# uncbiag/OAI_analysis_2

Hardware: AMD Instinct MI355X
Metric: knee MRI volumes/sec (segment+register), 384x384x160 fp32 (higher is better)
Workload: dtype fp16x3 (every fp32 value held as 2 fp16 terms = 22 mantissa bits, 3 MFMA passes per product, fp32 accumulate; fp32 in and out of every entry point; full-size parity vs the reference in `parity`)

## Files before the change

oai_analysis_2_amd/csrc/unet.hip:

```cpp
#include <cmath>
#include <cstdint>
#include <cstdlib>
#include <cstring>
#include <algorithm>
#include <vector>

#include "unet_host.h"
#include "unet_wino.h"

#ifdef OAI_DIAG
static unsigned long long* g_diag_stamps = nullptr;
static unsigned long long* diag_stamps() {
    if (!g_diag_stamps && oai::diag_env("OAI_STAMPS", 0)) {
        if (hipMalloc((void**)&g_diag_stamps, 32 * sizeof(unsigned long long)) != hipSuccess) return nullptr;
        (void)hipMemset(g_diag_stamps, 0, 32 * sizeof(unsigned long long));
    }
    return g_diag_stamps;
}
extern "C" int oai_diag_stamps(unsigned long long out[32], int reset) {
    if (!g_diag_stamps) return 1;
    if (hipMemcpy(out, g_diag_stamps, 32 * sizeof(unsigned long long), hipMemcpyDeviceToHost) != hipSuccess) return 2;
    if (reset) (void)hipMemset(g_diag_stamps, 0, 32 * sizeof(unsigned long long));
    return 0;
}
// ... 221 lines not shown
    return best;
}


int fill_conv_args(const oai_unet* h, const Layer& L, const float* s0, const float* s1, float* out, const int dims[3], const ConvOpt& o, ConvArgs& a) {
    if (o.head) a = *o.head;
    if (o.store_boxes && h->sres && h->opt_dead_stores) { a.store_boxes = o.store_boxes; a.store_grow = 1; }
    if (o.first) {
        a.first_w = h->L[EC0].plain; a.first_scale = h->L[EC0].scale_f16; a.first_shift = h->L[EC0].shift_f16; a.first_src = *o.first;
        a.first_census = census_of(h, EC0);
    }
    if (const Scatter* sc = o.sc) {
        a.sc_boxes = sc->boxes; a.sc_ntiles = sc->ntiles; a.sc_tile0 = sc->tile0;
        for (int i = 0; i < 3; ++i) { a.sc_g[i] = sc->g[i]; a.sc_e[i] = sc->e[i]; a.sc_t[i] = sc->t[i]; }
    }
    a.boxes = o.boxes;
    a.pool_out = o.pool_out;
    a.range_flag = h->range_flag;
#ifdef OAI_DIAG
    a.stamps = layer_stamps(h, L);
#endif
    a.src0 = s0; a.src1 = s1; a.C0 = L.c0; a.C1 = s1 ? L.c1 : 0;
    const bool f16 = h->precision == OAI_PREC_FP16X3;
    a.out = out; a.Cout = L.cout; a.scale = f16 ? L.scale_f16 : L.scale; a.shift = f16 ? L.shift_f16 : L.shift;
    a.census = h->sres ? census_of(h, layer_id(h, L)) : nullptr;
    a.wpanel = h->precision == OAI_PREC_F32 ? L.panel : L.panel_bf[h->precision == OAI_PREC_BF16X3 ? 0 : h->precision == OAI_PREC_BF16X6 ? 1 : 2];
    a.wpanel16 = h->precision == OAI_PREC_FP16X3 && layer_bit(h, h->opt_m16_layers, L) ? L.panel_m16 : nullptr;
    a.D = dims[0]; a.H = dims[1]; a.W = dims[2];
    a.ncb = (L.cout + 63) / 64;
    a.relu = 1;
// ... 9 lines not shown
    if (h->precision == OAI_PREC_F32 && h->variant == 0 && h->opt_wino_f32 && L.panel_wino_f32 && a.Cout % 4 == 0 && !a.head_w && !a.first_w && !a.sc_boxes &&
        (!a.pool_out || (wino_pool_box(box, dims) && dims[0] % 2 == 0)) && layer_bit(h, h->opt_wino_layers, L))
        return launch_conv3_wino_f32(h, L, a, box, ntiles, st);
    if (h->sres && h->opt_wino && L.panel_wino && h->sres_mrep == 4 && !a.first_w && !a.head_w && !a.sc_boxes &&
        (!a.pool_out || (a.Cout % 128 == 0 && a.relu && wino_pool_box(box, dims))) && a.Cout % 64 == 0 && (h->opt_wino & (a.Cout % 128 == 0 ? 1 : 2)) && (a.Cout % 128 == 0 || (a.C0 + 15) / 16 + (a.C1 + 15) / 16 >= 8) && layer_bit(h, h->opt_wino_layers, L) && (size_t)dims[0] * dims[1] * dims[2] < (1u << 24))
        return launch_conv3_wino(h, L, a, box, ntiles, st, o.oc);
    return launch_conv3_direct(h, a, box, ntiles, st);
}

static bool pool_fusable(const oai_unet* h, const int dims[3], const Box& box) {
    if (h->variant != 0) return false;
    for (int i = 0; i < 3; ++i) if (box.lo[i] != 0 || box.hi[i] != dims[i]) return false;
    return dims[0] % 4 == 0 && dims[1] % 8 == 0 && dims[2] % 16 == 0;
}


static int run_batch(oai_unet* h, const TileSource& src, int n, const Box need[18], int out_mode,
                     float* blocks_out, float* const buf[B_COUNT], hipStream_t st,
                     const int* table = nullptr, int table_tiles = 0, int t0 = 0, const SharedEnc* se = nullptr, const OwnPlan* own = nullptr) {
    auto tb = [&](int layer) -> const int* { return table ? table + ((size_t)layer * table_tiles + t0) * 6 : nullptr; };
    if (!table || !h->opt_own_cover) own = nullptr;
    OwnCover ocs[kOwnLayers];
    auto oc = [&](int layer) -> const OwnCover* {
        if (!own) return nullptr;
        const int slot = own_cover_slot(layer);
        ocs[slot].list = own->list[slot]; ocs[slot].list_len = own->list_len[slot];
        for (int s = 0; s < 3; ++s) {
            ocs[slot].rows[s] = tb(18 + 3 * slot + s);
            for (int i = 0; i < 3; ++i) ocs[slot].nb[s][i] = own->nb[slot][s][i];
            const int ncb = h->L[layer].cout / (64 * wino_groups(h, h->L[layer].cout, kWinoTY[s]));
            ocs[slot].xcd_group[s] = own->nb[slot][s][0] && ncb > 0 && !ocs[slot].list_len ? balanced_xcd_group(h->xcd_group, own->tile_nb.data() + (slot * 3 + s) * 3, n, own->nb[slot][s], ncb) : 0;
        }
        return &ocs[slot];
    };
    auto upv = [&](int layer) { return own ? own->up_nvox[layer] : 0; };
    const Layer* L = h->L;
    int d[4][3];
    for (int l = 0; l < 4; ++l) { d[l][0] = src.td >> l; d[l][1] = src.th >> l; d[l][2] = src.tw >> l; }

    int rc;
#define RUN(x) do { rc = (x); if (rc) return rc; } while (0)
    if (se) {
        {
            TileSource vs{};
            vs.vol = se->vol; vs.D = se->D; vs.H = se->H; vs.W = se->W; vs.td = se->PD; vs.th = se->PH; vs.tw = se->PW;
            vs.ez = se->PD; vs.ey = se->PH; vs.ex = se->PW; vs.oz = se->overlap[0]; vs.oy = se->overlap[1]; vs.ox = se->overlap[2]; vs.gy = 1; vs.gx = 1;
            const int per_row = se->grid[1] * se->grid[2], P[3] = {se->PD, se->PH, se->PW};
            Scatter sc;
            sc.boxes = tb(DC2); sc.ntiles = n; sc.tile0 = src.tile_begin;
            for (int i = 0; i < 3; ++i) { sc.g[i] = se->grid[i]; sc.e[i] = se->eff[i]; }
            sc.t[0] = src.td; sc.t[1] = src.th; sc.t[2] = src.tw;
            const int t_first = src.tile_begin, t_last = src.tile_begin + n - 1;
            const int zspan = (src.td + se->eff[0] - 1) / se->eff[0];
            const int s_first = t_first / per_row, s_last = t_last / per_row + zspan - 1;
            Box prev{}; bool have_prev = false;
            for (int s = s_first; s <= s_last; ++s) {
// ... 10 lines not shown
                if (jhi < 0) continue;
                Box bx;
                bx.lo[0] = se->eff[0] * s; bx.hi[0] = std::min(P[0], se->eff[0] * (s + 1));
                if (s == s_last) bx.hi[0] = std::min(P[0], se->eff[0] * (t_last / per_row) + src.td);
                bx.lo[1] = se->eff[1] * jlo; bx.hi[1] = std::min(P[1], se->eff[1] * jhi + src.th);
                bx.lo[2] = se->eff[2] * klo; bx.hi[2] = std::min(P[2], se->eff[2] * khi + src.tw);
                if (have_prev && prev.lo[1] == bx.lo[1] && prev.hi[1] == bx.hi[1] && prev.lo[2] == bx.lo[2] && prev.hi[2] == bx.hi[2] && prev.hi[0] == bx.lo[0]) {
                    prev.hi[0] = bx.hi[0];
                    continue;
                }
                if (have_prev) RUN(launch_conv3(h, L[EC1], nullptr, nullptr, buf[B_SYN0], P, prev, 1, st, {.pool_out = se->SP0, .first = &vs, .sc = &sc}));
                prev = bx; have_prev = true;
            }
            if (have_prev) RUN(launch_conv3(h, L[EC1], nullptr, nullptr, buf[B_SYN0], P, prev, 1, st, {.pool_out = se->SP0, .first = &vs, .sc = &sc}));
        }
        RUN(launch_pooled_gather(h, *se, src, buf[B_P0], d[1], n, st));
        RUN(launch_first_shell(h, src, buf[B_E0], d[0], n, st));
        const int td = d[0][0], th = d[0][1], tw = d[0][2];
        const Box zlo = {{0, 0, 0}, {2, th, tw}}, zhi = {{td - 2, 0, 0}, {td, th, tw}};
        const Box ylo = {{2, 0, 0}, {td - 2, 2, tw}}, yhi = {{2, th - 2, 0}, {td - 2, th, tw}};
        const Box xlo = {{2, 2, 0}, {td - 2, th - 2, 2}}, xhi = {{2, 2, tw - 2}, {td - 2, th - 2, tw}};
        const bool zpool = tb(EC1) != nullptr && h->opt_dead_stores;
        RUN((launch_conv3_one<16, 2, 4, 1>(h, L[EC1], buf[B_E0], buf[B_SYN0], d[0], zlo, n, st, tb(EC1), zpool ? buf[B_P0] : nullptr)));
        RUN((launch_conv3_one<16, 2, 4, 1>(h, L[EC1], buf[B_E0], buf[B_SYN0], d[0], zhi, n, st, tb(EC1), zpool ? buf[B_P0] : nullptr)));
        RUN((launch_conv3_one<16, 2, 1, 4>(h, L[EC1], buf[B_E0], buf[B_SYN0], d[0], ylo, n, st, tb(EC1))));
        RUN((launch_conv3_one<16, 2, 1, 4>(h, L[EC1], buf[B_E0], buf[B_SYN0], d[0], yhi, n, st, tb(EC1))));
        RUN((launch_conv3_one<2, 16, 4, 1>(h, L[EC1], buf[B_E0], buf[B_SYN0], d[0], xlo, n, st, tb(EC1))));
        RUN((launch_conv3_one<2, 16, 4, 1>(h, L[EC1], buf[B_E0], buf[B_SYN0], d[0], xhi, n, st, tb(EC1))));
        RUN(launch_pool(h, buf[B_SYN0], buf[B_P0], d[0], L[EC1].cout, n, st, zpool ? 2 : 1));
    } else {
    const bool fuse_first = first_fusable(h, need[EC1]);
    const TileSource* fsrc = fuse_first ? &src : nullptr;
    if (!fuse_first) RUN(launch_first(h, src, buf[B_E0], n, st));
    if (pool_fusable(h, d[0], need[EC1])) {
        RUN(launch_conv3(h, L[EC1], buf[B_E0], nullptr, buf[B_SYN0], d[0], need[EC1], n, st, {.boxes = tb(EC1), .pool_out = buf[B_P0], .first = fsrc, .store_boxes = tb(DC2)}));
    } else {
        RUN(launch_conv3(h, L[EC1], buf[B_E0], nullptr, buf[B_SYN0], d[0], need[EC1], n, st, {.boxes = tb(EC1), .first = fsrc}));
        RUN(launch_pool(h, buf[B_SYN0], buf[B_P0], d[0], L[EC1].cout, n, st));
    }
    }
    RUN(launch_conv3(h, L[EC2], buf[B_P0], nullptr, buf[B_E2], d[1], need[EC2], n, st, {.boxes = tb(EC2)}));
    if (pool_fusable(h, d[1], need[EC3])) {
        RUN(launch_conv3(h, L[EC3], buf[B_E2], nullptr, buf[B_SYN1], d[1], need[EC3], n, st, {.boxes = tb(EC3), .pool_out = buf[B_P1], .store_boxes = tb(DC5)}));
    } else {
        RUN(launch_conv3(h, L[EC3], buf[B_E2], nullptr, buf[B_SYN1], d[1], need[EC3], n, st, {.boxes = tb(EC3)}));
        RUN(launch_pool(h, buf[B_SYN1], buf[B_P1], d[1], L[EC3].cout, n, st));
    }
    RUN(launch_conv3(h, L[EC4], buf[B_P1], nullptr, buf[B_E4], d[2], need[EC4], n, st, {.boxes = tb(EC4)}));
    if (pool_fusable(h, d[2], need[EC5])) {
        RUN(launch_conv3(h, L[EC5], buf[B_E4], nullptr, buf[B_SYN2], d[2], need[EC5], n, st, {.boxes = tb(EC5), .pool_out = buf[B_P2], .store_boxes = tb(DC8)}));
    } else {
        RUN(launch_conv3(h, L[EC5], buf[B_E4], nullptr, buf[B_SYN2], d[2], need[EC5], n, st, {.boxes = tb(EC5)}));
        RUN(launch_pool(h, buf[B_SYN2], buf[B_P2], d[2], L[EC5].cout, n, st));
    }
    RUN(launch_conv3(h, L[EC6], buf[B_P2], nullptr, buf[B_E6], d[3], need[EC6], n, st, {.boxes = tb(EC6)}));
    RUN(launch_conv3(h, L[EC7], buf[B_E6], nullptr, buf[B_E7], d[3], need[EC7], n, st, {.boxes = tb(EC7)}));
// ... 150 lines not shown
            }
            if ((L.kind != 0 && L.kind != 1) || L.panel_bf[slot]) continue;
            if (int rc = upload(h, pack_conv3_panel_bf(L.wk_host, L.c0, L.c1, L.cout, NS), &L.panel_bf[slot])) return rc;
        }
        if (slot == 2 && !h->L[EC0].scale_f16)
            if (int rc = refresh_fp16_affine(h)) return rc;
    }
    h->precision = mode;
    h->sres = mode == OAI_PREC_FP16X3 && h->opt_sres;
    return OAI_OK;
}

struct IntOption { const char* name; int oai_unet::*field; int lo, hi; const char* message; };
static const IntOption kIntOptions[] = {
    {"shared_enc", &oai_unet::opt_shared, 0, 1, "oai_unet_set_option: shared_enc must be 0 or 1"},
    {"wide", &oai_unet::opt_wide, 0, 2, "oai_unet_set_option: wide must be 0, 1 or 2 (2 = also for launches of fewer than 1024 workgroups)"},
    {"winograd_layers", &oai_unet::opt_wino_layers, 0, 0x3FFFF, "oai_unet_set_option: winograd_layers is a mask over the 18 layers"},
    {"m16", &oai_unet::opt_m16, 0, 1, "oai_unet_set_option: m16 must be 0 or 1"},
    {"m16_layers", &oai_unet::opt_m16_layers, 0, 0x3FFFF, "oai_unet_set_option: m16_layers is a mask over the 18 layers"},
    {"dead_stores", &oai_unet::opt_dead_stores, 0, 1, "oai_unet_set_option: dead_stores must be 0 or 1"},
    {"winograd_f32", &oai_unet::opt_wino_f32, 0, 1, "oai_unet_set_option: winograd_f32 must be 0 or 1"},
    {"first_blocks", &oai_unet::opt_first_blocks, 1, 4096, "oai_unet_set_option: first_blocks must be in [1, 4096]"},
    {"up_nbw", &oai_unet::opt_up_nbw, 0, 64, "oai_unet_set_option: up_nbw must be in [0, 64]"},
    {"own_cover", &oai_unet::opt_own_cover, 0, 1, "oai_unet_set_option: own_cover must be 0 or 1"},
    {"one_launch", &oai_unet::opt_one_launch, 0, 7, "oai_unet_set_option: one_launch must be in [0, 7] (bit 0 two-group layers, bit 1 the 64-cout layer, bit 2 force)"},
    {"fuse_first", &oai_unet::fuse_first, 0, 1, "oai_unet_set_option: fuse_first must be 0 or 1"},
    {"xcd_group", &oai_unet::xcd_group, 0, 4096, "oai_unet_set_option: xcd_group must be in [0, 4096]"},
};

int oai_unet_set_option(oai_unet* h, const char* name, int value) {
// ... 557 lines not shown
```

oai_analysis_2_amd/csrc/unet_direct.hip:

```cpp
#include "unet_host.h"
#include "unet_sres2.h"

namespace oai {

template <int RX, int RY, int WY, int WX, int V = 0>
static void launch_sres2(int var, unsigned grid, hipStream_t st, const ConvArgs& a, const unsigned char* zero_rec) {
#ifdef OAI_DIAG
    if constexpr (V < 10)
        if (var != V) return launch_sres2<RX, RY, WY, WX, V + 1>(var, grid, st, a, zero_rec);
#endif
    conv3_igemm_sres2<RX, RY, WY, WX, V><<<grid, 512, 0, st>>>(a, zero_rec);
}

template <int MREP, int KC, int RX, int RY, int WY, int WX>
static int launch_conv3_shape(const oai_unet* h, ConvArgs a, const Box& box, int ntiles, hipStream_t st, int mrep_override = 0) {
    for (int i = 0; i < 3; ++i) { a.lo[i] = box.lo[i]; a.hi[i] = box.hi[i]; }
    if (box.hi[0] <= box.lo[0] || box.hi[1] <= box.lo[1] || box.hi[2] <= box.lo[2]) return OAI_OK;
    const int sres_mrep = mrep_override ? mrep_override : h->sres_mrep;
    constexpr bool kMainShape = RX == 16 && RY == 2 && WY == 4 && WX == 1;
    constexpr bool kWideShape = kMainShape || (RX == 16 && RY == 2 && WY == 2 && WX == 2);
    bool wide = KC == 8 && kWideShape && h->sres && h->opt_wide && sres_mrep == 4 && !a.first_w && !a.head_w && a.Cout % 128 == 0;
    if (wide && h->opt_wide == 1) {
        const size_t nwg = (size_t)ntiles * cdiv(box.hi[0] - box.lo[0], 4) * cdiv(box.hi[1] - box.lo[1], WY * RY) * cdiv(box.hi[2] - box.lo[2], WX * RX) * (a.Cout / 128);
        wide = nwg >= (kMainShape ? 1024 : 512);
    }
    if (wide) a.ncb = a.Cout / 128;
    const bool bf = KC == 8 && h->precision != OAI_PREC_F32;
    constexpr int kF32Mrep = MREP > 2 ? 2 : MREP;
    a.nbz = cdiv(box.hi[0] - box.lo[0], bf ? (h->sres ? sres_mrep : 2) : kF32Mrep);
    a.nby = cdiv(box.hi[1] - box.lo[1], WY * RY);
    a.nbx = cdiv(box.hi[2] - box.lo[2], WX * RX);
    unsigned grid = (unsigned)((size_t)ntiles * a.nbz * a.nby * a.nbx * a.ncb);
    if (KC == 8 && h->sres) grid = xcd_deal(h, grid, a.nblocks, a.xcd_group);
    if (int rc = launch_begin(h, st)) return rc;
    if (KC == 8 && h->sres) {
        static const int one_wg = diag_env("OAI_ONE_WG", 0);
        bool done = false;
        const bool m16 = h->opt_m16 && a.wpanel16 && a.Cout % 128 != 0 && !one_wg;
        if (m16) a.wpanel = a.wpanel16;
        if constexpr (RX == 16 && RY == 2 && WY == 4 && WX == 1) {
            if (a.first_w) {
                if (m16) launch_sres_m16<RX, RY, WY, WX>(4, true, grid, st, a, h->zero_rec);
                else conv3_igemm_sres<4, RX, RY, WY, WX, true><<<grid, 256, 0, st>>>(a, h->zero_rec);
                done = true;
            }
        }
        if constexpr (kWideShape) {
            if (wide) {
                static const int var = diag_env("OAI_WIDE_VAR", 0);
                launch_sres2<RX, RY, WY, WX>(var >= 1 && var <= 10 ? var : 0, grid, st, a, h->zero_rec);
                done = true;
            }
        }
        if (done) { }
        else if (a.first_w) return set_error(OAI_ERR_ARG, "fused ec0 asked of a tile shape that has no such kernel");
        else if (m16) launch_sres_m16<RX, RY, WY, WX>(sres_mrep, false, grid, st, a, h->zero_rec);
        else if (sres_mrep == 4) conv3_igemm_sres<4, RX, RY, WY, WX><<<grid, 256, one_wg ? 24 * 1024 : 0, st>>>(a, h->zero_rec);
        else conv3_igemm_sres<2, RX, RY, WY, WX><<<grid, 256, 0, st>>>(a, h->zero_rec);
    }
    else if (KC == 8 && h->precision == OAI_PREC_BF16X3) conv3_igemm_bf16s<2, false, 2, RX, RY, WY, WX><<<grid, 256, 0, st>>>(a);
    else if (KC == 8 && h->precision == OAI_PREC_BF16X6) conv3_igemm_bf16s<3, false, 2, RX, RY, WY, WX><<<grid, 256, 0, st>>>(a);
    else if (KC == 8 && h->precision == OAI_PREC_FP16X3) conv3_igemm_bf16s<2, true, 2, RX, RY, WY, WX><<<grid, 256, 0, st>>>(a);
    else conv3_igemm_f32<kF32Mrep, KC, RX, RY, WY, WX><<<grid, 256, 0, st>>>(a);
    return launch_end(h, st);
}

static Cover direct_cover(const oai_unet* h, const Box& box) { return cover_box(box, 16, 4, 8, h->variant == 2); }

bool first_fusion_ok(const oai_unet* h) {
    return h->sres && h->fuse_first && h->variant == 0 && h->sres_mrep == 4 && h->L[EC0].cout == 32 && h->L[EC1].c0 == 32;
}
bool first_fusable(const oai_unet* h, const Box& ec1_box) {
    if (!first_fusion_ok(h)) return false;
    const Cover c = direct_cover(h, ec1_box);
    return c.hr == 0 && c.wr == 0;
}

template <int RX, int RY, int WY, int WX>
int launch_conv3_one(const oai_unet* h, const Layer& L, const float* s0, float* out, const int dims[3], const Box& box, int ntiles,
                     hipStream_t st, const int* boxes, float* pool_only) {
    ConvArgs a;
    if (int rc = fill_conv_args(h, L, s0, nullptr, out, dims, {.boxes = boxes, .pool_out = pool_only}, a)) return rc;
    if (pool_only) { a.store_boxes = boxes; a.store_grow = -(1 << 20); }
    return launch_conv3_shape<4, 8, RX, RY, WY, WX>(h, a, box, ntiles, st, pool_only ? 2 : 0);
}
template int launch_conv3_one<16, 2, 4, 1>(const oai_unet*, const Layer&, const float*, float*, const int[3], const Box&, int, hipStream_t, const int*, float*);
template int launch_conv3_one<16, 2, 1, 4>(const oai_unet*, const Layer&, const float*, float*, const int[3], const Box&, int, hipStream_t, const int*, float*);
template int launch_conv3_one<2, 16, 4, 1>(const oai_unet*, const Layer&, const float*, float*, const int[3], const Box&, int, hipStream_t, const int*, float*);

int launch_conv3_direct(const oai_unet* h, const ConvArgs& a, const Box& box, int ntiles, hipStream_t st) {
#ifdef OAI_DIAG
    if (h->variant == 1) return launch_conv3_shape<2, 16, 16, 2, 4, 1>(h, a, box, ntiles, st);
#endif
    const Cover c = direct_cover(h, box);
    if (int rc = launch_conv3_shape<4, 8, 16, 2, 4, 1>(h, a, c.main, ntiles, st)) return rc;
    if (c.wr) {
        const int rc = c.wr <= 2 ? launch_conv3_shape<4, 8, 2, 16, 4, 1>(h, a, c.xs, ntiles, st)
                     : c.wr <= 4 ? launch_conv3_shape<4, 8, 4, 8, 4, 1>(h, a, c.xs, ntiles, st)
                                 : launch_conv3_shape<4, 8, 8, 4, 4, 1>(h, a, c.xs, ntiles, st);
// ... 8 lines not shown
```

oai_analysis_2_amd/csrc/unet_direct_m16.hip:

```cpp
#include "unet_host.h"
#include "unet_sres.h"

namespace oai {

template <int RX, int RY, int WY, int WX>
void launch_sres_m16(int mrep, bool first, unsigned grid, hipStream_t st, const ConvArgs& a, const unsigned char* zero_rec) {
    if constexpr (RX == 16 && RY == 2 && WY == 4 && WX == 1) {
        if (first) {
            conv3_igemm_sres<4, RX, RY, WY, WX, true, true><<<grid, 256, 0, st>>>(a, zero_rec);
            return;
        }
    }
    if (mrep == 4) conv3_igemm_sres<4, RX, RY, WY, WX, false, true><<<grid, 256, 0, st>>>(a, zero_rec);
    else conv3_igemm_sres<2, RX, RY, WY, WX, false, true><<<grid, 256, 0, st>>>(a, zero_rec);
}
template void launch_sres_m16<16, 2, 4, 1>(int, bool, unsigned, hipStream_t, const ConvArgs&, const unsigned char*);
template void launch_sres_m16<2, 16, 4, 1>(int, bool, unsigned, hipStream_t, const ConvArgs&, const unsigned char*);
template void launch_sres_m16<4, 8, 4, 1>(int, bool, unsigned, hipStream_t, const ConvArgs&, const unsigned char*);
template void launch_sres_m16<8, 4, 4, 1>(int, bool, unsigned, hipStream_t, const ConvArgs&, const unsigned char*);
template void launch_sres_m16<16, 2, 1, 4>(int, bool, unsigned, hipStream_t, const ConvArgs&, const unsigned char*);
template void launch_sres_m16<16, 2, 2, 2>(int, bool, unsigned, hipStream_t, const ConvArgs&, const unsigned char*);

}
```

oai_analysis_2_amd/csrc/unet_host.h:

```cpp
#pragma once
#include <algorithm>
#include <vector>

#include "common.h"
#include "unet_kernels.h"

namespace oai {

enum LayerId { EC0, EC1, EC2, EC3, EC4, EC5, EC6, EC7, DC9, DC8, DC7, DC6, DC5, DC4, DC3, DC2, DC1, DC0 };
__host__ __device__ static inline int layer_level(int k) { const int v[18] = {0, 0, 1, 1, 2, 2, 3, 3, 2, 2, 2, 1, 1, 1, 0, 0, 0, 0}; return v[k]; }
__host__ __device__ static inline int layer_kind(int k) { const int v[18] = {0, 0, 0, 0, 0, 0, 0, 0, 2, 1, 1, 2, 1, 1, 2, 1, 1, 3}; return v[k]; }

struct Layer {
    int kind = 0, cin = 0, cout = 0;
    int c0 = 0, c1 = 0;
    float4* panel = nullptr;
    float4* panel_bf[3] = {nullptr, nullptr, nullptr};
    float* scale_f16 = nullptr;
    float* shift_f16 = nullptr;
    float* plain_f16 = nullptr;
    std::vector<float> ws;
    int rel1 = 0;
    size_t panel_f16_floats = 0;
    float4* panel_wino_f32 = nullptr;
// ... 15 lines not shown
struct oai_unet {
    oai::Layer L[18];
    int variant = 0;
    int precision = OAI_PREC_F32;
    int* range_flag = nullptr;
    unsigned* census = nullptr;
    int* eval_out = nullptr;
    int act_exp[18] = {0};
    bool calibrated = false;
    int opt_wino_f32 = 1;
    int opt_first_blocks = 24;
    int opt_up_nbw = 0;
    int opt_own_cover = 1;
    int opt_one_launch = 1;
    int opt_shared = 1;
    int opt_wide = 1;
    int opt_wino = 19;
    int opt_wino_layers = 0x3FFFF;
    int opt_m16 = 1;
    int opt_m16_layers = 0x3FFFF;
    int opt_dead_stores = 1;
    int opt_census = 1;
    int xcd_group = 32;
    int fuse_first = 1;
    int sres_mrep = 4;
    bool opt_sres = true;
    bool sres = false;
    unsigned char* zero_rec = nullptr;
    int n_classes = 0;
    std::vector<void*> allocs;
// ... 34 lines not shown
struct SharedEnc {
    float* SP0;
    int PD, PH, PW;
    const float* vol; int D, H, W;
    int grid[3], eff[3], overlap[3];
};

struct ConvOpt {
    const int* boxes = nullptr;
    float* pool_out = nullptr;
    const ConvArgs* head = nullptr;
    const TileSource* first = nullptr;
    const int* store_boxes = nullptr;
    const Scatter* sc = nullptr;
    const OwnCover* oc = nullptr;
};

static inline int layer_src0(int k) { return k - 1; }
static inline int layer_src1(int k) { return k == DC8 ? EC5 : k == DC5 ? EC3 : k == DC2 ? EC1 : -1; }

static inline int layer_id(const oai_unet* h, const Layer& L) { return (int)(&L - h->L); }
static inline bool layer_bit(const oai_unet* h, int mask, const Layer& L) { return (mask >> layer_id(h, L)) & 1; }
static inline unsigned* census_of(const oai_unet* h, int k) { return h->opt_census ? h->census + 16 * k : nullptr; }

static inline unsigned capped_blocks(size_t total, size_t cap) { return (unsigned)std::min<size_t>((total + 255) / 256, cap); }

int launch_begin(const oai_unet* h, hipStream_t st);
int launch_end(const oai_unet* h, hipStream_t st);
unsigned xcd_deal(const oai_unet* h, unsigned grid, int& nblocks, int& xcd_group, int group = 0);
int fill_conv_args(const oai_unet* h, const Layer& L, const float* s0, const float* s1, float* out, const int dims[3], const ConvOpt& o, ConvArgs& a);
// ... 50 lines not shown
```

oai_analysis_2_amd/csrc/unet_kernels.h:

```cpp
#pragma once
#include <hip/hip_runtime.h>

namespace oai {

typedef float f32x16 __attribute__((ext_vector_type(16)));


struct TileSource {
    const float* vol;
    const float* tiles;
    int D, H, W;
    int td, th, tw;
    int ez, ey, ex;
    int oz, oy, ox;
    int gy, gx;
    int tile_begin;
};

__device__ __forceinline__ int reflect_index(int v, int n) {
    const int p = 2 * (n - 1);
    int m = v % p;
    if (m < 0) m += p;
    return m < n ? m : p - m;
}
// ... 20 lines not shown
    unsigned* census = nullptr;
    unsigned* first_census = nullptr;
    int own_origin = 0;
    unsigned long long* stamps = nullptr;
    int nblocks = 0, xcd_group = 0;
    int* reserved1 = nullptr;
    const float* head_w = nullptr;
    const float* head_b = nullptr;
    const int* head_boxes = nullptr;
    float* head_out = nullptr;
    int head_ncls = 0, head_mode = 0;
    int head_k[3] = {0, 0, 0}, head_e[3] = {0, 0, 0};
    const float* first_w = nullptr;
    const float* first_scale = nullptr; const float* first_shift = nullptr;
    TileSource first_src = {};
};

__device__ __forceinline__ int xcd_block_id(int nblocks, int G) {
    const int xcd = (int)blockIdx.x & 7, j = (int)blockIdx.x >> 3;
    const int id = ((j / G) * 8 + xcd) * G + j % G;
    return id < nblocks ? id : -1;
}

__device__ __forceinline__ bool tile_box(const int* boxes, int tile, const int (&llo)[3], const int (&lhi)[3],
                                         int (&lo)[3], int (&hi)[3]) {
#pragma unroll
    for (int i = 0; i < 3; ++i) { lo[i] = llo[i]; hi[i] = lhi[i]; }
    if (boxes) {
        const int* b = boxes + 6 * tile;
#pragma unroll
// ... 755 lines not shown
```

oai_analysis_2_amd/csrc/unet_sres.h:

```cpp
#pragma once
#include <hip/hip_runtime.h>

#include <type_traits>

#include "unet_kernels.h"

namespace oai {

typedef unsigned short u16x8 __attribute__((ext_vector_type(8)));

__device__ __forceinline__ unsigned split2_f16(float x, unsigned& lo_bits) {
    const _Float16 h = (_Float16)x;
    const _Float16 l = (_Float16)(x - (float)h);
    lo_bits = __builtin_bit_cast(unsigned short, l);
    return __builtin_bit_cast(unsigned short, h);
}

__device__ __forceinline__ float join2_f16(unsigned short hi, unsigned short lo) {
    return (float)__builtin_bit_cast(_Float16, hi) + (float)__builtin_bit_cast(_Float16, lo);
}

__device__ __forceinline__ unsigned census_peek(const unsigned* census) {
    typedef const __attribute__((address_space(4))) unsigned* cuptr;
    return census ? *((cuptr)census + (blockIdx.x & 15)) : 0u;
// ... 78 lines not shown
        *reinterpret_cast<u16x4*>(o + q * 8) = hi;
        *reinterpret_cast<u16x4*>(o + 32 + q * 8) = lo;
    }
}
#endif

typedef float f32x4m __attribute__((ext_vector_type(4)));
typedef _Float16 f16x8m __attribute__((ext_vector_type(8)));
template <int IMM>
__device__ __forceinline__ f32x4m gload16m(const void* sbase, unsigned voff) {
    f32x4m v;
    asm volatile("global_load_dwordx4 %0, %1, %2 offset:%3" : "=v"(v) : "v"(voff), "s"(sbase), "n"(IMM) : "memory");
    return v;
}

template <int MREP, int RX, int RY, int WY, int WX, bool FIRST = false, bool M16 = false>
__global__ void __launch_bounds__(256, MREP == 2 ? 3 : 2) conv3_igemm_sres(const ConvArgs a, const unsigned char* __restrict__ zero_rec) {
    static_assert(RX * RY == 32 && WY * WX == 4 && (MREP == 2 || MREP == 4), "bad tile shape");
    constexpr int NREP = 2, TZ = MREP;
    constexpr int kTY = WY * RY, kTX = WX * RX, HY = kTY + 2, HX = kTX + 2, HZ = TZ + 2;
    constexpr int HVOX = HZ * HY * HX;
    constexpr int PIECES = HVOX * 4;
    constexpr int NIT = (PIECES + 255) / 256;
    constexpr int BUF = NIT * 256 * 16;
    __shared__ __attribute__((aligned(16))) unsigned char lds[BUF];
    constexpr int PZ = HZ + 2, PY = HY + 2, PX = HX + 2;
    __shared__ float raw[FIRST ? PZ * PY * PX : 1];
    __shared__ int rawidx[FIRST ? PZ + PY + PX : 1];

    const int tid = threadIdx.x, lane = tid & 63, wave = tid >> 6;
    int id = a.xcd_group ? xcd_block_id(a.nblocks, a.xcd_group) : (int)blockIdx.x;
    if (id < 0) return;
    const int cb = id % a.ncb; id /= a.ncb;
// ... 48 lines not shown
        else return acc[m][n][r];
    };
    const int col16 = lane & 15, rq16 = lane >> 4;
    auto row_of = [&](int r) __attribute__((always_inline)) -> int {
        return M16 ? 16 * (r >> 3) + 4 * rq16 + (r & 3) : (r & 3) + 8 * (r >> 2) + 4 * (lane >> 5);
    };

    const int nch0 = (a.C0 + 15) / 16, nch1 = (a.C1 + 15) / 16, nchunks = nch0 + nch1;
    const size_t plane = (size_t)a.D * a.H * a.W;
    const unsigned char* s0 = reinterpret_cast<const unsigned char*>(a.src0) + srec(tile, nch0, plane, 0, 0);
    const unsigned char* s1 = reinterpret_cast<const unsigned char*>(a.src1) + srec(tile, nch1, plane, 0, 0);

    constexpr unsigned kNoPiece = 0xFFFFFFFFu;
    unsigned poff[NIT];
    const int pslot = tid & 3;
#pragma unroll
    for (int it = 0; it < (FIRST ? 0 : NIT); ++it) {
        const int r = (it * 256 + tid) >> 2;
        const int hx = r % HX, t2 = r / HX, hy = t2 % HY, hz = t2 / HY;
        const int gz = oz0 - 1 + hz, gy = oy0 - 1 + hy, gx = ox0 - 1 + hx;
        const bool ok = r < HVOX && (unsigned)gz < (unsigned)a.D && (unsigned)gy < (unsigned)a.H && (unsigned)gx < (unsigned)a.W;
        poff[it] = ok ? ((unsigned)((gz * a.H + gy) * a.W + gx) << 6) | (unsigned)((pslot ^ ((hx >> 2) & 3)) << 4) : kNoPiece;
    }
    auto stage = [&](int ch) __attribute__((always_inline)) {
        const bool first = ch < nch0;
        const unsigned char* cb = (first ? s0 : s1) + (size_t)(first ? ch : ch - nch0) * plane * 64;
#pragma unroll
        for (int it = 0; it < NIT; ++it) {
            const unsigned char* g = poff[it] != kNoPiece ? cb + poff[it] : zero_rec;
            __builtin_amdgcn_global_load_lds((const __attribute__((address_space(1))) void*)g,
                                             (__attribute__((address_space(3))) void*)(lds + (it * 256 + wave * 64) * 16), 16, 0, 0);
        }
    };

    float first_max = 0.0f;
    if constexpr (FIRST) {
        const TileSource& s = a.first_src;
        if (tid < PZ + PY + PX) {
            const int ax = tid < PZ ? 0 : tid < PZ + PY ? 1 : 2;
            const int p = tid - (ax == 0 ? 0 : ax == 1 ? PZ : PZ + PY);
            const int c = (ax == 0 ? oz0 : ax == 1 ? oy0 : ox0) - 2 + p;
            const int tdim = ax == 0 ? s.td : ax == 1 ? s.th : s.tw;
            int v = -1;
            if ((unsigned)c < (unsigned)tdim) {
// ... 482 lines not shown
            for (int it = 0; it < EIT; ++it) {
                constexpr int kDummy = 0; (void)kDummy;
                const int c = (it & 3) * 32, zc = it >> 2;
                const int xc = kWide ? c % kTX : 0, yc = c / kTX;
                const int oz = oz0 + zc, oy = oyl + yc, ox = oxl + xc;
                if (cok && oz >= clo[0] && oz < chi[0] && oy >= clo[1] && oy < chi[1] && ox >= clo[2] && ox < chi[2]) {
                    const unsigned uni = (unsigned)(((oz * a.H + oy0 + yc) * a.W + ox0 + xc) * 64);
                    float4* dstp = reinterpret_cast<float4*>(ob + (size_t)(lane_off + uni));
                    const float4 val = *reinterpret_cast<const float4*>(lds + (it * 256 + tid) * 16);
                    __builtin_nontemporal_store(val.x, &dstp->x); __builtin_nontemporal_store(val.y, &dstp->y);
                    __builtin_nontemporal_store(val.z, &dstp->z); __builtin_nontemporal_store(val.w, &dstp->w);
                }
            }
        }
        OAI_STAMPB(head ? 4 : 3);
        if constexpr (RX == 16 && RY == 2 && WY == 4 && WX == 1) {
            if (a.pool_out) {
                unsigned char* pb = reinterpret_cast<unsigned char*>(a.pool_out);
                const int Dp = a.D / 2, Hp = a.H / 2, Wp = a.W / 2;
                const bool relu = a.relu != 0;
                auto val = [&](int m, int r) {
                    const float v = acc_el(m, n, r) * scv[n][M16 ? (r >> 2) & 1 : 0] + shv[n][M16 ? (r >> 2) & 1 : 0];
                    return relu ? fmaxf(v, 0.0f) : v;
                };
#pragma unroll
                for (int g = 0; g < 2; ++g)
#pragma unroll
                    for (int p = 0; p < 2; ++p) {
                        const int r0 = 4 * g + 2 * p;
#pragma unroll
                        for (int m = 0; m < MREP; m += 2) {
                            float v = fmaxf(fmaxf(val(m, r0), val(m, r0 + 1)), fmaxf(val(m, r0 + 8), val(m, r0 + 9)));
                            v = fmaxf(v, fmaxf(fmaxf(val(m + 1, r0), val(m + 1, r0 + 1)), fmaxf(val(m + 1, r0 + 8), val(m + 1, r0 + 9))));
                            const int x = M16 ? ox0 + 4 * rq16 + 2 * p : ox0 + 8 * g + 4 * half + 2 * p, y = oy0 + 2 * wy, z = oz0 + m;
                            const int pco = M16 ? cb * 64 + n * 32 + 16 * g + col16 : co;
                            store_split_pair(pb + srec(tile, nco, (size_t)Dp * Hp * Wp, 0, (((size_t)(z / 2)) * Hp + y / 2) * Wp + x / 2), (size_t)Dp * Hp * Wp * 64,
                                             pco, v, M16 ? (g ? cvalid1 : cvalid) : cvalid, a.range_flag);
                        }
                    }
            }
        }
    }
    OAI_STAMPB(5);
    if (head) {
        int hlo[3], hhi[3];
        tile_box(a.head_boxes, tile, blo, bhi, hlo, hhi);
        const size_t evox = (size_t)a.head_e[0] * a.head_e[1] * a.head_e[2];
#pragma unroll
        for (int j = 0; j < HV; ++j) {
            const int vox = j * 256 + tid;
            const int oz = oz0 + vox / (kTX * kTY), oy = oy0 + (vox / kTX) % kTY, ox = ox0 + vox % kTX;
            if (oz >= hlo[0] && oz < hhi[0] && oy >= hlo[1] && oy < hhi[1] && ox >= hlo[2] && ox < hhi[2]) {
                const size_t o = ((size_t)(oz - a.head_k[0]) * a.head_e[1] + (oy - a.head_k[1])) * a.head_e[2] + (ox - a.head_k[2]);
#pragma unroll
// ... 12 lines not shown
    }
    if constexpr (FIRST) census_note(a.first_census, a.range_flag, first_max, seen_first);
    census_note(a.census, a.range_flag, vmax, seen);
#ifdef OAI_DIAG
    OAI_STAMP(6);
    OAI_STAMPB(6);
    if (a.stamps && lane == 0) {
        for (int i = 0; i < 8; ++i) atomicAdd(a.stamps + i, (unsigned long long)st_sum[i]);
        atomicAdd(a.stamps + 8, 1ull);
        atomicAdd(a.stamps + 9, (unsigned long long)st_chunks);
    }
#endif
#undef OAI_STAMP
#undef OAI_STAMPB
#undef OAI_STAMP_
}

#ifdef OAI_UNET_PLAIN_KERNELS
__global__ void __launch_bounds__(256, 2) upconv2_igemm_sres(const UpArgs a) {
#ifdef OAI_DIAG
    unsigned ust[5] = {0, 0, 0, 0, 0};
    unsigned long long ulast = __builtin_amdgcn_s_memtime();
#define OAI_USTAMP(i) do { if (a.stamps) { const unsigned long long now_ = __builtin_amdgcn_s_memtime(); ust[i] += (unsigned)(now_ - ulast); ulast = now_; } } while (0)
#else
#define OAI_USTAMP(i) do { } while (0)
#endif
    constexpr int kStage = 24 * 1024, kRing = 3 * kStage;
    __shared__ __attribute__((aligned(16))) unsigned char ulds[kRing + 512];
    const int tid = threadIdx.x, lane = tid & 63, wave = tid >> 6;
    const int wm = wave >> 1, wn = wave & 1;
// ... 470 lines not shown
```

Before: 7.949.

## Read pooled shared volume in place for ec2 and pool y/x faces in epilogue

In the shared-encoder path, the ec2 conv can now read interior voxels directly from the shared pooled volume through a per-tile view offset, instead of first gathering them into a per-tile buffer. Only face voxels still come from the tile buffer. The y and x face launches of ec1 also max-pool in their epilogue, which removes the separate pool launch. Together this cuts a gather kernel, a pool kernel and their memory traffic, at the cost of per-load branching on the address source and a new kernel variant.

```diff
diff --git a/oai_analysis_2_amd/csrc/unet.hip b/oai_analysis_2_amd/csrc/unet.hip
--- a/oai_analysis_2_amd/csrc/unet.hip
+++ b/oai_analysis_2_amd/csrc/unet.hip
@@ -259,6 +259,12 @@
         a.sc_boxes = sc->boxes; a.sc_ntiles = sc->ntiles; a.sc_tile0 = sc->tile0;
         for (int i = 0; i < 3; ++i) { a.sc_g[i] = sc->g[i]; a.sc_e[i] = sc->e[i]; a.sc_t[i] = sc->t[i]; }
     }
+    if (const SharedEnc* se = o.view) {
+        a.view = se->SP0; a.view_tile0 = o.view_tile0;
+        a.view_dim[0] = se->PD / 2; a.view_dim[1] = se->PH / 2; a.view_dim[2] = se->PW / 2;
+        for (int i = 0; i < 3; ++i) a.view_e[i] = se->eff[i] / 2;
+        a.view_g[0] = se->grid[1]; a.view_g[1] = se->grid[2];
+    }
     a.boxes = o.boxes;
     a.pool_out = o.pool_out;
     a.range_flag = h->range_flag;
@@ -298,6 +304,10 @@
     return dims[0] % 4 == 0 && dims[1] % 8 == 0 && dims[2] % 16 == 0;
 }
 
+static bool view_layer_ok(const oai_unet* h, const Layer& L) {
+    return (h->opt_shared_view & 1) && h->sres && h->sres_mrep == 4 && L.c1 == 0 && L.cout % 128 != 0 && (L.c0 + 15) / 16 < 8;
+}
+
 
 static int run_batch(oai_unet* h, const TileSource& src, int n, const Box need[18], int out_mode,
                      float* blocks_out, float* const buf[B_COUNT], hipStream_t st,
@@ -324,6 +334,7 @@
 
     int rc;
 #define RUN(x) do { rc = (x); if (rc) return rc; } while (0)
+    const SharedEnc* view = nullptr;
     if (se) {
         {
             TileSource vs{};
@@ -364,7 +375,8 @@
             }
             if (have_prev) RUN(launch_conv3(h, L[EC1], nullptr, nullptr, buf[B_SYN0], P, prev, 1, st, {.pool_out = se->SP0, .first = &vs, .sc = &sc}));
         }
-        RUN(launch_pooled_gather(h, *se, src, buf[B_P0], d[1], n, st));
+        view = view_layer_ok(h, L[EC2]) ? se : nullptr;
+        if (!view) RUN(launch_pooled_gather(h, *se, src, buf[B_P0], d[1], n, st));
         RUN(launch_first_shell(h, src, buf[B_E0], d[0], n, st));
         const int td = d[0][0], th = d[0][1], tw = d[0][2];
         const Box zlo = {{0, 0, 0}, {2, th, tw}}, zhi = {{td - 2, 0, 0}, {td, th, tw}};
@@ -373,11 +385,12 @@
         const bool zpool = tb(EC1) != nullptr && h->opt_dead_stores;
         RUN((launch_conv3_one<16, 2, 4, 1>(h, L[EC1], buf[B_E0], buf[B_SYN0], d[0], zlo, n, st, tb(EC1), zpool ? buf[B_P0] : nullptr)));
         RUN((launch_conv3_one<16, 2, 4, 1>(h, L[EC1], buf[B_E0], buf[B_SYN0], d[0], zhi, n, st, tb(EC1), zpool ? buf[B_P0] : nullptr)));
-        RUN((launch_conv3_one<16, 2, 1, 4>(h, L[EC1], buf[B_E0], buf[B_SYN0], d[0], ylo, n, st, tb(EC1))));
-        RUN((launch_conv3_one<16, 2, 1, 4>(h, L[EC1], buf[B_E0], buf[B_SYN0], d[0], yhi, n, st, tb(EC1))));
-        RUN((launch_conv3_one<2, 16, 4, 1>(h, L[EC1], buf[B_E0], buf[B_SYN0], d[0], xlo, n, st, tb(EC1))));
-        RUN((launch_conv3_one<2, 16, 4, 1>(h, L[EC1], buf[B_E0], buf[B_SYN0], d[0], xhi, n, st, tb(EC1))));
-        RUN(launch_pool(h, buf[B_SYN0], buf[B_P0], d[0], L[EC1].cout, n, st, zpool ? 2 : 1));
+        float* const yxpool = zpool && (h->opt_shared_view & 2) ? buf[B_P0] : nullptr;
+        RUN((launch_conv3_one<16, 2, 1, 4>(h, L[EC1], buf[B_E0], buf[B_SYN0], d[0], ylo, n, st, tb(EC1), yxpool)));
+        RUN((launch_conv3_one<16, 2, 1, 4>(h, L[EC1], buf[B_E0], buf[B_SYN0], d[0], yhi, n, st, tb(EC1), yxpool)));
+        RUN((launch_conv3_one<2, 16, 4, 1>(h, L[EC1], buf[B_E0], buf[B_SYN0], d[0], xlo, n, st, tb(EC1), yxpool)));
+        RUN((launch_conv3_one<2, 16, 4, 1>(h, L[EC1], buf[B_E0], buf[B_SYN0], d[0], xhi, n, st, tb(EC1), yxpool)));
+        if (!yxpool) RUN(launch_pool(h, buf[B_SYN0], buf[B_P0], d[0], L[EC1].cout, n, st, zpool ? 2 : 1));
     } else {
     const bool fuse_first = first_fusable(h, need[EC1]);
     const TileSource* fsrc = fuse_first ? &src : nullptr;
@@ -389,7 +402,7 @@
         RUN(launch_pool(h, buf[B_SYN0], buf[B_P0], d[0], L[EC1].cout, n, st));
     }
     }
-    RUN(launch_conv3(h, L[EC2], buf[B_P0], nullptr, buf[B_E2], d[1], need[EC2], n, st, {.boxes = tb(EC2)}));
+    RUN(launch_conv3(h, L[EC2], buf[B_P0], nullptr, buf[B_E2], d[1], need[EC2], n, st, {.boxes = tb(EC2), .view = view, .view_tile0 = src.tile_begin}));
     if (pool_fusable(h, d[1], need[EC3])) {
         RUN(launch_conv3(h, L[EC3], buf[B_E2], nullptr, buf[B_SYN1], d[1], need[EC3], n, st, {.boxes = tb(EC3), .pool_out = buf[B_P1], .store_boxes = tb(DC5)}));
     } else {
@@ -570,6 +583,7 @@
 struct IntOption { const char* name; int oai_unet::*field; int lo, hi; const char* message; };
 static const IntOption kIntOptions[] = {
     {"shared_enc", &oai_unet::opt_shared, 0, 1, "oai_unet_set_option: shared_enc must be 0 or 1"},
+    {"shared_view", &oai_unet::opt_shared_view, 0, 3, "oai_unet_set_option: shared_view must be in [0, 3] (bit 0 ec2 reads the pooled volume in place, bit 1 the y and x faces pool in their epilogue)"},
     {"wide", &oai_unet::opt_wide, 0, 2, "oai_unet_set_option: wide must be 0, 1 or 2 (2 = also for launches of fewer than 1024 workgroups)"},
     {"winograd_layers", &oai_unet::opt_wino_layers, 0, 0x3FFFF, "oai_unet_set_option: winograd_layers is a mask over the 18 layers"},
     {"m16", &oai_unet::opt_m16, 0, 1, "oai_unet_set_option: m16 must be 0 or 1"},
diff --git a/oai_analysis_2_amd/csrc/unet_direct.hip b/oai_analysis_2_amd/csrc/unet_direct.hip
--- a/oai_analysis_2_amd/csrc/unet_direct.hip
+++ b/oai_analysis_2_amd/csrc/unet_direct.hip
@@ -25,6 +25,8 @@
         wide = nwg >= (kMainShape ? 1024 : 512);
     }
     if (wide) a.ncb = a.Cout / 128;
+    if (a.view && (KC != 8 || !h->sres || wide || a.first_w || sres_mrep != 4 || a.C1))
+        return set_error(OAI_ERR_ARG, "an in-place view of the pooled volume asked of a launch that has no such kernel");
     const bool bf = KC == 8 && h->precision != OAI_PREC_F32;
     constexpr int kF32Mrep = MREP > 2 ? 2 : MREP;
     a.nbz = cdiv(box.hi[0] - box.lo[0], bf ? (h->sres ? sres_mrep : 2) : kF32Mrep);
@@ -55,6 +57,7 @@
         if (done) { }
         else if (a.first_w) return set_error(OAI_ERR_ARG, "fused ec0 asked of a tile shape that has no such kernel");
         else if (m16) launch_sres_m16<RX, RY, WY, WX>(sres_mrep, false, grid, st, a, h->zero_rec);
+        else if (a.view) conv3_igemm_sres_view<4, RX, RY, WY, WX, false><<<grid, 256, 0, st>>>(a, h->zero_rec);
         else if (sres_mrep == 4) conv3_igemm_sres<4, RX, RY, WY, WX><<<grid, 256, one_wg ? 24 * 1024 : 0, st>>>(a, h->zero_rec);
         else conv3_igemm_sres<2, RX, RY, WY, WX><<<grid, 256, 0, st>>>(a, h->zero_rec);
     }
@@ -82,7 +85,7 @@
     ConvArgs a;
     if (int rc = fill_conv_args(h, L, s0, nullptr, out, dims, {.boxes = boxes, .pool_out = pool_only}, a)) return rc;
     if (pool_only) { a.store_boxes = boxes; a.store_grow = -(1 << 20); }
-    return launch_conv3_shape<4, 8, RX, RY, WY, WX>(h, a, box, ntiles, st, pool_only ? 2 : 0);
+    return launch_conv3_shape<4, 8, RX, RY, WY, WX>(h, a, box, ntiles, st, pool_only && box.hi[0] - box.lo[0] == 2 ? 2 : 0);
 }
 template int launch_conv3_one<16, 2, 4, 1>(const oai_unet*, const Layer&, const float*, float*, const int[3], const Box&, int, hipStream_t, const int*, float*);
 template int launch_conv3_one<16, 2, 1, 4>(const oai_unet*, const Layer&, const float*, float*, const int[3], const Box&, int, hipStream_t, const int*, float*);
diff --git a/oai_analysis_2_amd/csrc/unet_direct_m16.hip b/oai_analysis_2_amd/csrc/unet_direct_m16.hip
--- a/oai_analysis_2_amd/csrc/unet_direct_m16.hip
+++ b/oai_analysis_2_amd/csrc/unet_direct_m16.hip
@@ -11,7 +11,8 @@
             return;
         }
     }
-    if (mrep == 4) conv3_igemm_sres<4, RX, RY, WY, WX, false, true><<<grid, 256, 0, st>>>(a, zero_rec);
+    if (a.view) conv3_igemm_sres_view<4, RX, RY, WY, WX, true><<<grid, 256, 0, st>>>(a, zero_rec);
+    else if (mrep == 4) conv3_igemm_sres<4, RX, RY, WY, WX, false, true><<<grid, 256, 0, st>>>(a, zero_rec);
     else conv3_igemm_sres<2, RX, RY, WY, WX, false, true><<<grid, 256, 0, st>>>(a, zero_rec);
 }
 template void launch_sres_m16<16, 2, 4, 1>(int, bool, unsigned, hipStream_t, const ConvArgs&, const unsigned char*);
diff --git a/oai_analysis_2_amd/csrc/unet_host.h b/oai_analysis_2_amd/csrc/unet_host.h
--- a/oai_analysis_2_amd/csrc/unet_host.h
+++ b/oai_analysis_2_amd/csrc/unet_host.h
@@ -53,6 +53,7 @@
     int opt_own_cover = 1;
     int opt_one_launch = 1;
     int opt_shared = 1;
+    int opt_shared_view = 1;
     int opt_wide = 1;
     int opt_wino = 19;
     int opt_wino_layers = 0x3FFFF;
@@ -117,6 +118,8 @@
     const int* store_boxes = nullptr;
     const Scatter* sc = nullptr;
     const OwnCover* oc = nullptr;
+    const SharedEnc* view = nullptr;
+    int view_tile0 = 0;
 };
 
 static inline int layer_src0(int k) { return k - 1; }
diff --git a/oai_analysis_2_amd/csrc/unet_kernels.h b/oai_analysis_2_amd/csrc/unet_kernels.h
--- a/oai_analysis_2_amd/csrc/unet_kernels.h
+++ b/oai_analysis_2_amd/csrc/unet_kernels.h
@@ -58,6 +58,8 @@
     const float* first_w = nullptr;
     const float* first_scale = nullptr; const float* first_shift = nullptr;
     TileSource first_src = {};
+    const float* view = nullptr;
+    int view_dim[3] = {0, 0, 0}, view_e[3] = {0, 0, 0}, view_g[2] = {0, 0}, view_tile0 = 0;
 };
 
 __device__ __forceinline__ int xcd_block_id(int nblocks, int G) {
diff --git a/oai_analysis_2_amd/csrc/unet_sres.h b/oai_analysis_2_amd/csrc/unet_sres.h
--- a/oai_analysis_2_amd/csrc/unet_sres.h
+++ b/oai_analysis_2_amd/csrc/unet_sres.h
@@ -116,9 +116,10 @@
     return v;
 }
 
-template <int MREP, int RX, int RY, int WY, int WX, bool FIRST = false, bool M16 = false>
-__global__ void __launch_bounds__(256, MREP == 2 ? 3 : 2) conv3_igemm_sres(const ConvArgs a, const unsigned char* __restrict__ zero_rec) {
+template <int MREP, int RX, int RY, int WY, int WX, bool FIRST, bool M16, bool VIEW>
+__device__ __forceinline__ void conv3_igemm_sres_body(const ConvArgs& a, const unsigned char* __restrict__ zero_rec) {
     static_assert(RX * RY == 32 && WY * WX == 4 && (MREP == 2 || MREP == 4), "bad tile shape");
+    static_assert(!(VIEW && FIRST), "the view is a way of reading an input tensor: FIRST reads none");
     constexpr int NREP = 2, TZ = MREP;
     constexpr int kTY = WY * RY, kTX = WX * RX, HY = kTY + 2, HX = kTX + 2, HZ = TZ + 2;
     constexpr int HVOX = HZ * HY * HX;
@@ -197,20 +198,32 @@
     constexpr unsigned kNoPiece = 0xFFFFFFFFu;
     unsigned poff[NIT];
     const int pslot = tid & 3;
+    unsigned vorg = 0;
+    if constexpr (VIEW) {
+        const int t = a.view_tile0 + tile;
+        const int tk = t % a.view_g[1], tj = (t / a.view_g[1]) % a.view_g[0], ti = t / (a.view_g[0] * a.view_g[1]);
+        vorg = (unsigned)((ti * a.view_e[0] * a.view_dim[1] + tj * a.view_e[1]) * a.view_dim[2] + tk * a.view_e[2]);
+    }
 #pragma unroll
     for (int it = 0; it < (FIRST ? 0 : NIT); ++it) {
         const int r = (it * 256 + tid) >> 2;
         const int hx = r % HX, t2 = r / HX, hy = t2 % HY, hz = t2 / HY;
         const int gz = oz0 - 1 + hz, gy = oy0 - 1 + hy, gx = ox0 - 1 + hx;
         const bool ok = r < HVOX && (unsigned)gz < (unsigned)a.D && (unsigned)gy < (unsigned)a.H && (unsigned)gx < (unsigned)a.W;
-        poff[it] = ok ? ((unsigned)((gz * a.H + gy) * a.W + gx) << 6) | (unsigned)((pslot ^ ((hx >> 2) & 3)) << 4) : kNoPiece;
+        unsigned vox = (unsigned)((gz * a.H + gy) * a.W + gx), from_view = 0u;
+        if constexpr (VIEW) {
+            const bool face = gz == 0 || gz == a.D - 1 || gy == 0 || gy == a.H - 1 || gx == 0 || gx == a.W - 1;
+            if (!face) { vox = vorg + (unsigned)((gz * a.view_dim[1] + gy) * a.view_dim[2] + gx); from_view = 1u; }
+        }
+        poff[it] = ok ? (vox << 6) | (unsigned)((pslot ^ ((hx >> 2) & 3)) << 4) | from_view : kNoPiece;
     }
     auto stage = [&](int ch) __attribute__((always_inline)) {
         const bool first = ch < nch0;
         const unsigned char* cb = (first ? s0 : s1) + (size_t)(first ? ch : ch - nch0) * plane * 64;
+        const unsigned char* cbv = VIEW ? reinterpret_cast<const unsigned char*>(a.view) + (size_t)ch * a.view_dim[0] * a.view_dim[1] * a.view_dim[2] * 64 - 1 : nullptr;
 #pragma unroll
         for (int it = 0; it < NIT; ++it) {
-            const unsigned char* g = poff[it] != kNoPiece ? cb + poff[it] : zero_rec;
+            const unsigned char* g = poff[it] != kNoPiece ? (VIEW && (poff[it] & 1u) ? cbv : cb) + poff[it] : zero_rec;
             __builtin_amdgcn_global_load_lds((const __attribute__((address_space(1))) void*)g,
                                              (__attribute__((address_space(3))) void*)(lds + (it * 256 + wave * 64) * 16), 16, 0, 0);
         }
@@ -723,7 +736,9 @@
             }
         }
         OAI_STAMPB(head ? 4 : 3);
-        if constexpr (RX == 16 && RY == 2 && WY == 4 && WX == 1) {
+        constexpr bool kPoolMain = RX == 16 && RY == 2 && WY == 4 && WX == 1, kPoolYFace = !VIEW && RX == 16 && RY == 2 && WY == 1 && WX == 4;
+        constexpr bool kPoolXFace = !VIEW && RX == 2 && RY == 16 && WY == 4 && WX == 1;
+        if constexpr (kPoolMain || kPoolYFace || kPoolXFace) {
             if (a.pool_out) {
                 unsigned char* pb = reinterpret_cast<unsigned char*>(a.pool_out);
                 const int Dp = a.D / 2, Hp = a.H / 2, Wp = a.W / 2;
@@ -732,6 +747,10 @@
                     const float v = acc_el(m, n, r) * scv[n][M16 ? (r >> 2) & 1 : 0] + shv[n][M16 ? (r >> 2) & 1 : 0];
                     return relu ? fmaxf(v, 0.0f) : v;
                 };
+                auto live = [&](int m, int r0) {
+                    return kPoolMain || (((okmask >> r0) & 1u) != 0 && oz0 + m >= blo[0] && oz0 + m < bhi[0]);
+                };
+                if constexpr (!kPoolXFace) {
 #pragma unroll
                 for (int g = 0; g < 2; ++g)
 #pragma unroll
@@ -741,12 +760,27 @@
                         for (int m = 0; m < MREP; m += 2) {
                             float v = fmaxf(fmaxf(val(m, r0), val(m, r0 + 1)), fmaxf(val(m, r0 + 8), val(m, r0 + 9)));
                             v = fmaxf(v, fmaxf(fmaxf(val(m + 1, r0), val(m + 1, r0 + 1)), fmaxf(val(m + 1, r0 + 8), val(m + 1, r0 + 9))));
-                            const int x = M16 ? ox0 + 4 * rq16 + 2 * p : ox0 + 8 * g + 4 * half + 2 * p, y = oy0 + 2 * wy, z = oz0 + m;
+                            const int x = ox0 + wx * RX + (M16 ? 4 * rq16 + 2 * p : 8 * g + 4 * half + 2 * p), y = oy0 + RY * wy, z = oz0 + m;
                             const int pco = M16 ? cb * 64 + n * 32 + 16 * g + col16 : co;
                             store_split_pair(pb + srec(tile, nco, (size_t)Dp * Hp * Wp, 0, (((size_t)(z / 2)) * Hp + y / 2) * Wp + x / 2), (size_t)Dp * Hp * Wp * 64,
-                                             pco, v, M16 ? (g ? cvalid1 : cvalid) : cvalid, a.range_flag);
+                                             pco, v, (M16 ? (g ? cvalid1 : cvalid) : cvalid) && live(m, r0), a.range_flag);
                         }
                     }
+                } else {
+#pragma unroll
+                for (int k = 0; k < 4; ++k) {
+                    const int r0 = 4 * k;
+#pragma unroll
+                    for (int m = 0; m < MREP; m += 2) {
+                        float v = fmaxf(fmaxf(val(m, r0), val(m, r0 + 1)), fmaxf(val(m, r0 + 2), val(m, r0 + 3)));
+                        v = fmaxf(v, fmaxf(fmaxf(val(m + 1, r0), val(m + 1, r0 + 1)), fmaxf(val(m + 1, r0 + 2), val(m + 1, r0 + 3))));
+                        const int x = ox0, y = oy0 + wy * RY + (M16 ? 8 * (k >> 1) + 2 * rq16 : 4 * k + 2 * half), z = oz0 + m;
+                        const int pco = M16 ? cb * 64 + n * 32 + 16 * (k & 1) + col16 : co;
+                        store_split_pair(pb + srec(tile, nco, (size_t)Dp * Hp * Wp, 0, (((size_t)(z / 2)) * Hp + y / 2) * Wp + x / 2), (size_t)Dp * Hp * Wp * 64,
+                                         pco, v, (M16 ? ((k & 1) ? cvalid1 : cvalid) : cvalid) && live(m, r0), a.range_flag);
+                    }
+                }
+                }
             }
         }
     }
@@ -789,6 +823,15 @@
 #undef OAI_STAMP
 #undef OAI_STAMPB
 #undef OAI_STAMP_
+}
+
+template <int MREP, int RX, int RY, int WY, int WX, bool FIRST = false, bool M16 = false>
+__global__ void __launch_bounds__(256, MREP == 2 ? 3 : 2) conv3_igemm_sres(const ConvArgs a, const unsigned char* __restrict__ zero_rec) {
+    conv3_igemm_sres_body<MREP, RX, RY, WY, WX, FIRST, M16, false>(a, zero_rec);
+}
+template <int MREP, int RX, int RY, int WY, int WX, bool M16>
+__global__ void __launch_bounds__(256, MREP == 2 ? 3 : 2) conv3_igemm_sres_view(const ConvArgs a, const unsigned char* __restrict__ zero_rec) {
+    conv3_igemm_sres_body<MREP, RX, RY, WY, WX, false, M16, true>(a, zero_rec);
 }
 
 #ifdef OAI_UNET_PLAIN_KERNELS
```

After: 8.010 (median of 6 runs). About the same (+0.8%).
